# LCSL/nys-koop-lqr

Measured on AMD Instinct MI355X. Metric: Nyström-Koopman fits/sec (K_nm build + A,B,C solve), N=1e5 m=2000 d=384, higher is better.
Workload: dtype f64

## Files before the change

### nys_koop_lqr_amd/csrc/nk_api.hip

```cpp
#include "nk_common.h"

#include <cmath>
#include <cstdarg>
#include <cstdio>
#include <cstring>
#include <chrono>
#include <cstdlib>
#include <algorithm>
#include <condition_variable>
#include <mutex>
#include <set>
#include <thread>

namespace nk {

static thread_local std::string g_err;

void set_error(const char* fmt, ...) {
  char buf[1024];
  va_list ap;
  va_start(ap, fmt);
  vsnprintf(buf, sizeof(buf), fmt, ap);
  va_end(ap);
  g_err = buf;
// ... 792 lines not shown
        nk_model_destroy(m);
      }
    }
  } guard{ctx, mdl};
  mdl->ktype = kd->type; mdl->sigma0 = kd->sigma0; mdl->jitter = jitter;

  tr.mark("validate + model_alloc");
  hipEvent_t* ev = ctx->ev;
  NK_HIP(hipEventRecord(ev[0], ctx->stream));
  NK_TRY(make_winv(ctx, kd, d, mdl->winv));
  MatIn x, y, zi, zo;
  int host_passes = 1;
  if (mode != FIT_SOLVE) {
    const char* e = getenv("NYSKOOP_HOST_PASSES");
    const int want = e ? atoi(e) : 6;
    if (want > 1 && rng.size() == 2 && !ctx_recording(ctx) && (double)n_eff * (2.0 * d + p) * 8.0 >= 64e6 &&
        !is_device_ptr(X) && !is_device_ptr(Y))
      host_passes = want > 8 ? 8 : want;
  }
  if (mode != FIT_SOLVE && host_passes > 1) {
    x.ld = (d + p + 1) & ~(int64_t)1;
    y.ld = (d + 1) & ~(int64_t)1;
    double *xd = nullptr, *yd = nullptr;
    NK_TRY(arena_alloc_t(ctx, (size_t)n * x.ld, &xd));
    NK_TRY(arena_alloc_t(ctx, (size_t)n * y.ld, &yd));
    x.ptr = xd; y.ptr = yd; x.staged = y.staged = true;
  } else if (mode != FIT_SOLVE) {
    NK_TRY(stage_in(ctx, X, ldx, n, d + p, &x));
    NK_TRY(stage_in(ctx, Y, ldy, n, d, &y));
  }
  if (mode != FIT_SOLVE && rng.size() > 2 && (double)n_eff * (2.0 * d + p) * 8.0 <= 256e6) {
    const int64_t ldxg = (d + p + 1) & ~(int64_t)1, ldyg = (d + 1) & ~(int64_t)1;
    double *xg = nullptr, *yg = nullptr;
    NK_TRY(arena_alloc_t(ctx, (size_t)n_eff * ldxg, &xg));
    NK_TRY(arena_alloc_t(ctx, (size_t)n_eff * ldyg, &yg));
    int64_t o = 0;
    for (size_t i = 0; i < rng.size(); i += 2) {
      const int64_t b = rng[i], len = rng[i + 1] - rng[i];
      NK_TRY(launch_copy2d(ctx, x.ptr + b * x.ld, x.ld, xg + o * ldxg, ldxg, len, d + p));
      NK_TRY(launch_copy2d(ctx, y.ptr + b * y.ld, y.ld, yg + o * ldyg, ldyg, len, d));
      o += len;
    }
    x.ptr = xg; x.ld = ldxg; y.ptr = yg; y.ld = ldyg;
    rng.assign({(int64_t)0, n_eff});
  }
  NK_TRY(stage_in(ctx, Zout, ldzo, m, d, &zo));
  if (same_centers) zi = zo; else NK_TRY(stage_in(ctx, Zin, ldzi, m, d, &zi));
  NK_TRY(launch_copy2d(ctx, zo.ptr, zo.ld, mdl->Z, d, m, d));
  NK_HIP(hipEventRecord(ev[1], ctx->stream));
  tr.mark("staging issued");

  double *Kmm = nullptr, *Kj = nullptr, *Kj_in = nullptr, *Kxo = nullptr;
  bool landmarks_aside = false;
  if (mode != FIT_GRAM) {
  NK_TRY(arena_alloc_t(ctx, (size_t)m * m, &Kmm));
  NK_TRY(arena_alloc_t(ctx, (size_t)m * m, &Kj));
  if (same_centers) {
    Kj_in = Kj;
    Kxo = Kmm;
  } else {
    NK_TRY(arena_alloc_t(ctx, (size_t)m * m, &Kj_in));
    NK_TRY(arena_alloc_t(ctx, (size_t)m * m, &Kxo));
  }
  {
    const char* la = getenv("NYSKOOP_LANDMARKS_ASIDE");
    landmarks_aside = mode == FIT_FULL && n_eff >= 20000 && m >= 1024 && !ctx_recording(ctx) && !(la && la[0] == '0');
  }
  {
    hipStream_t s0 = ctx->stream;
    if (landmarks_aside) {
      NK_HIP(hipEventRecord(ev[12], ctx->stream));
      ctx->stream = ctx->stream_prep;
      NK_HIP(hipStreamWaitEvent(ctx->stream, ev[12], 0));
    }
    int rc_l = launch_kmat(ctx, kd->type, zo.ptr, zo.ld, m, zo.ptr, zo.ld, m, d, mdl->winv, kd->sigma0, Kmm, m);
    if (rc_l == NK_OK) rc_l = launch_copy2d(ctx, Kmm, m, Kj, m, m, m);
    if (rc_l == NK_OK) rc_l = launch_add_diag(ctx, Kj, m, m, jitter);
    if (rc_l == NK_OK && !same_centers) {
      rc_l = launch_kmat(ctx, kd->type, zi.ptr, zi.ld, m, zi.ptr, zi.ld, m, d, mdl->winv, kd->sigma0, Kj_in, m);
      if (rc_l == NK_OK) rc_l = launch_add_diag(ctx, Kj_in, m, m, jitter);
      if (rc_l == NK_OK) rc_l = launch_kmat(ctx, kd->type, zi.ptr, zi.ld, m, zo.ptr, zo.ld, m, d, mdl->winv, kd->sigma0, Kxo, m);
    }
    const hipError_t he = rc_l == NK_OK ? hipEventRecord(ev[8], ctx->stream) : hipSuccess;
    ctx->stream = s0;
    NK_TRY(rc_l);
    NK_HIP(he);
  }
  }
  double *G1 = nullptr, *G2 = nullptr, *G3 = nullptr, *G4 = nullptr;
  const int64_t ldd = d + (d & 1);
  NK_TRY(arena_alloc_t(ctx, gram_doubles(m, d, p), &G1));
  G2 = G1 + (size_t)mp * mp;
  G3 = G1 + gram_block1(m, p);
  G4 = G3 + (size_t)m * m;
  float ms_gram_kernel = 0.f;
  int gram_launches = 0;
  bool gram_deferred = false;
  const bool timed = stats != nullptr;
  SqrtPlan splan;
  int it = 0;
  double resid = 0.0;
  double *Sinvt = nullptr, *T1t = nullptr, *X1 = nullptr;
  auto alloc_sqrt_bufs = [&]() -> int {
    if (Sinvt == nullptr) NK_TRY(arena_alloc_t(ctx, (size_t)m * m, &Sinvt));
    if (T1t == nullptr) NK_TRY(arena_alloc_t(ctx, (size_t)m * m, &T1t));
    if (X1 == nullptr) NK_TRY(arena_alloc_t(ctx, (size_t)m * m, &X1));
    return NK_OK;
  };
  auto sqrt_products = [&]() -> int {
    NK_TRY(launch_transpose(ctx, mdl->Sinv, m, Sinvt, m, m, m));
    if (same_centers) {
      NK_TRY(launch_copy2d(ctx, mdl->S, m, T1t, m, m, m));
      NK_TRY(launch_axpby2d(ctx, -jitter, mdl->Sinv, m, 1.0, T1t, m, m, m));
    } else {
      NK_TRY(launch_transpose(ctx, Kxo, m, X1, m, m, m));
      NK_TRY(launch_gemm(ctx, true, false, m, m, m, 1.0, X1, m, mdl->Sinv, m, 0.0, T1t, m));
    }
    return NK_OK;
  };
  auto queue_prep = [&]() -> int {
    SideScope prep(ctx, ctx->stream_prep);
    NK_HIP(hipStreamWaitEvent(ctx->stream, ev[8], 0));
    splan.lambda_min_hint = jitter > 0.0 ? jitter : 0.0;
    if (mode == FIT_FULL && n_eff >= 20000 && m >= 1024) {
      static const double frac = getenv("NYSKOOP_PREP_PAUSE") ? atof(getenv("NYSKOOP_PREP_PAUSE")) : 0.0;
      const int nb = (m + CHOL_NB - 1) / CHOL_NB;
      if (frac < 1.0) {
        splan.pause_event = ctx->ev_fork;
        splan.pause_step = std::max(0, std::min(nb - 1, (int)(frac * nb)));
      }
    }
    NK_TRY(sqrtm_prepare(ctx, Kj, m, m, &splan));
    NK_HIP(hipEventRecord(ev[9], ctx->stream));
    return NK_OK;
  };
  auto queue_side = [&]() -> int {
    NK_TRY(alloc_sqrt_bufs());
    SideScope side(ctx);
    NK_HIP(hipStreamWaitEvent(ctx->stream, ctx->ev_fork, 0));
    NK_HIP(hipStreamWaitEvent(ctx->stream, ev[9], 0));
    NK_HIP(hipEventRecord(ev[6], ctx->stream));
    NK_TRY(sqrtm_finish(ctx, &splan, mdl->S, mdl->Sinv));
    NK_HIP(hipEventRecord(ev[7], ctx->stream));
    NK_TRY(sqrt_products());
    NK_HIP(hipEventRecord(ctx->ev_join, ctx->stream));
    return NK_OK;
  };
  if (mode == FIT_SOLVE) {
    NK_HIP(hipMemcpyAsync(G1, gram_io, gram_doubles(m, d, p) * sizeof(double),
                          is_device_ptr(gram_io) ? hipMemcpyDeviceToDevice : hipMemcpyHostToDevice, ctx->stream));
    NK_HIP(hipEventRecord(ev[2], ctx->stream));
  } else {
  const bool f32 = ctx->compute_f32 != 0 && ctx->kmat_mode == 0 && d >= 32 && !ctx_recording(ctx) && m >= 4 && d >= 4;
  const int64_t off_out = f32 ? ((mp + 3) & ~3) : ((mp + 1) & ~1);
  const int64_t ldf = f32 ? ((off_out + m + 3) & ~(int64_t)3) : ((off_out + m + 1) & ~(int64_t)1);
  const double felem = f32 ? 4.0 : 8.0;
  int64_t pass_rows;
  {
    const char* b = getenv("NYSKOOP_F_BUDGET_GB");
    const double budget = (b ? atof(b) : 48.0) * 1073741824.0;
    pass_rows = (int64_t)(budget / ((double)ldf * felem));
    if (pass_rows < 1024) pass_rows = 1024;
    pass_rows &= ~(int64_t)1023;
    if (host_passes > 1) {
      const int64_t per = ((n_eff + host_passes - 1) / host_passes + 1023) & ~(int64_t)1023;
      if (per < pass_rows) pass_rows = per;
    }
  }
  struct Piece { int64_t b, len; };
  std::vector<std::vector<Piece>> passes(1);
  {
    int64_t used = 0;
    for (size_t i = 0; i < rng.size(); i += 2) {
      int64_t b = rng[i];
      const int64_t e = rng[i + 1];
      while (b < e) {
        if (used == pass_rows) { passes.emplace_back(); used = 0; }
        const int64_t len = std::min(e - b, pass_rows - used);
        passes.back().push_back(Piece{b, len});
        used += len;
        b += len;
      }
    }
  }
  const int64_t f_rows = passes.size() > 1 ? pass_rows : n_eff;
  double* F = nullptr;
  NK_TRY(arena_alloc_t(ctx, f32 ? ((size_t)f_rows * ldf + 1) / 2 + 64 : (size_t)f_rows * ldf + 64, &F));
  const bool gram_form = ctx->kmat_mode == 0 && d >= 32;
  int64_t maxlen = 0;
  for (auto& ps : passes) for (auto& pc : ps) maxlen = std::max(maxlen, pc.len);
  const int64_t ldt = (maxlen + 1) & ~(int64_t)1, ldzt = (m + 1) & ~1;
  double *center = nullptr, *Rt = nullptr, *sqr = nullptr, *Zto = nullptr, *sqzo = nullptr, *Zti = nullptr, *sqzi = nullptr;
  double *Rt2 = nullptr, *sqr2 = nullptr;
  const bool overlap_prep = gram_form && passes.size() == 1 && passes[0].size() == 1;
  if (gram_form) {
    NK_TRY(arena_alloc_t(ctx, (size_t)d, &center));
    if (!f32) {
      NK_TRY(arena_alloc_t(ctx, (size_t)d * ldt, &Rt));
      NK_TRY(arena_alloc_t(ctx, (size_t)maxlen, &sqr));
    }
    if (overlap_prep && !f32) {
      NK_TRY(arena_alloc_t(ctx, (size_t)d * ldt, &Rt2));
      NK_TRY(arena_alloc_t(ctx, (size_t)maxlen, &sqr2));
    }
    NK_TRY(arena_alloc_t(ctx, (size_t)d * ldzt, &Zto));
    NK_TRY(arena_alloc_t(ctx, (size_t)m, &sqzo));
    if (kd->type == NK_KERNEL_LINEAR) NK_TRY(launch_fill(ctx, center, d, 1, d, 0.0));
    else NK_TRY(launch_colmean(ctx, zo.ptr, zo.ld, m, d, center));
    NK_TRY(prep_rows(ctx, zo.ptr, zo.ld, m, d, mdl->winv, center, Zto, ldzt, sqzo));
    if (same_centers) {
      Zti = Zto; sqzi = sqzo;
    } else {
      NK_TRY(arena_alloc_t(ctx, (size_t)d * ldzt, &Zti));
      NK_TRY(arena_alloc_t(ctx, (size_t)m, &sqzi));
      NK_TRY(prep_rows(ctx, zi.ptr, zi.ld, m, d, mdl->winv, center, Zti, ldzt, sqzi));
    }
  }
  float *F32 = reinterpret_cast<float*>(F), *Rt32 = nullptr, *sq32 = nullptr, *Zt32 = nullptr, *sqz32 = nullptr, *Y32 = nullptr;
  const int64_t ldt32 = (maxlen + 3) & ~(int64_t)3, ldzt32 = (m + 3) & ~3, ldy32 = (d + 3) & ~3;
  if (f32) {
    NK_REQUIRE(same_centers, "fp32 engine: separate input landmarks are not supported");
    double* tmp = nullptr;
    NK_TRY(arena_alloc_t(ctx, ((size_t)d * ldt32 + 1) / 2 + 2, &tmp)); Rt32 = reinterpret_cast<float*>(tmp);
    NK_TRY(arena_alloc_t(ctx, ((size_t)maxlen + 1) / 2 + 2, &tmp)); sq32 = reinterpret_cast<float*>(tmp);
    NK_TRY(arena_alloc_t(ctx, ((size_t)d * ldzt32 + 1) / 2 + 2, &tmp)); Zt32 = reinterpret_cast<float*>(tmp);
    NK_TRY(arena_alloc_t(ctx, ((size_t)m + 1) / 2 + 2, &tmp)); sqz32 = reinterpret_cast<float*>(tmp);
    NK_TRY(arena_alloc_t(ctx, ((size_t)f_rows * ldy32 + 1) / 2 + 2, &tmp)); Y32 = reinterpret_cast<float*>(tmp);
    NK_TRY(prep_rows_f32(ctx, zo.ptr, zo.ld, m, d, mdl->winv, center, Zt32, ldzt32, sqz32));
  }
  const bool multi_pass = passes.size() > 1;
  const bool pipelined = host_passes > 1;
  auto upload_pass = [&](size_t ip) -> int {
    for (const Piece& pc : passes[ip]) {
      NK_HIP(hipMemcpy2DAsync(const_cast<double*>(x.ptr) + pc.b * x.ld, (size_t)x.ld * 8, X + pc.b * ldx, (size_t)ldx * 8,
                              (size_t)(d + p) * 8, (size_t)pc.len, hipMemcpyHostToDevice, ctx->stream_side));
      NK_HIP(hipMemcpy2DAsync(const_cast<double*>(y.ptr) + pc.b * y.ld, (size_t)y.ld * 8, Y + pc.b * ldy, (size_t)ldy * 8,
                              (size_t)d * 8, (size_t)pc.len, hipMemcpyHostToDevice, ctx->stream_side));
    }
    NK_HIP(hipEventRecord(ctx->ev_up[ip & 7], ctx->stream_side));
    return NK_OK;
  };
  if (pipelined) {
    NK_HIP(hipEventRecord(ev[12], ctx->stream));
    NK_HIP(hipStreamWaitEvent(ctx->stream_side, ev[12], 0));
    NK_TRY(upload_pass(0));
  }
  for (size_t ip = 0; ip < passes.size(); ++ip) {
    const std::vector<Piece>& ps = passes[ip];
    const double beta = ip == 0 ? 0.0 : 1.0;
    if (pipelined) NK_HIP(hipStreamWaitEvent(ctx->stream, ctx->ev_up[ip & 7], 0));
    if (f32) {
      int64_t o32 = 0;
      for (const Piece& pc : ps) {
        const double* xs = x.ptr + pc.b * x.ld;
        const double* ys = y.ptr + pc.b * y.ld;
        NK_TRY(prep_rows_f32(ctx, xs, x.ld, pc.len, d, mdl->winv, center, Rt32, ldt32, sq32));
        NK_TRY(launch_kmat_gram_f32(ctx, kd->type, Rt32, ldt32, sq32, pc.len, Zt32, ldzt32, sqz32, m, d, kd->sigma0,
                                    F32 + o32 * ldf, ldf));
        NK_TRY(prep_rows_f32(ctx, ys, y.ld, pc.len, d, mdl->winv, center, Rt32, ldt32, sq32));
        NK_TRY(launch_kmat_gram_f32(ctx, kd->type, Rt32, ldt32, sq32, pc.len, Zt32, ldzt32, sqz32, m, d, kd->sigma0,
                                    F32 + o32 * ldf + off_out, ldf));
        if (p > 0) NK_TRY(launch_cvt_f64_f32(ctx, xs + d, x.ld, F32 + o32 * ldf + m, ldf, pc.len, p));
        NK_TRY(launch_cvt_f64_f32(ctx, ys, y.ld, Y32 + o32 * ldy32, ldy32, pc.len, d));
        o32 += pc.len;
      }
      if (ip == 0) {
        NK_HIP(hipEventRecord(ev[2], ctx->stream));
        tr.mark("kmat issued");
      }
      TnProblemF pf[4];
      pf[0].A = F32; pf[0].B = F32; pf[0].lda = pf[0].ldb = ldf; pf[0].M = pf[0].N = mp; pf[0].C = G1; pf[0].ldc = mp;
      pf[0].tri = TRI_UPPER_MIRROR;
      pf[1].A = F32 + off_out; pf[1].B = F32; pf[1].lda = pf[1].ldb = ldf; pf[1].M = m; pf[1].N = mp; pf[1].C = G2; pf[1].ldc = mp;
      pf[2].A = F32 + off_out; pf[2].B = F32 + off_out; pf[2].lda = pf[2].ldb = ldf; pf[2].M = pf[2].N = m; pf[2].C = G3;
      pf[2].ldc = m; pf[2].tri = TRI_UPPER_MIRROR;
      pf[3].A = Y32; pf[3].lda = ldy32; pf[3].M = d; pf[3].N = m; pf[3].C = G4; pf[3].ldc = m; pf[3].B = F32 + off_out;
      pf[3].ldb = ldf;
      for (int q = 0; q < 4; ++q) pf[q].beta = beta;
      float ms1 = 0.f;
      NK_TRY(launch_gemm_tn_f32_multi(ctx, pf, 4, o32, 0, timed ? &ms1 : nullptr, multi_pass));
      if (multi_pass) ms_gram_kernel += ms1; else gram_deferred = timed;
      gram_launches += 1;
      if (pipelined && ip + 1 < passes.size()) NK_TRY(upload_pass(ip + 1));
      continue;
    }
    int64_t o = 0;
    for (const Piece& pc : ps) {
      const double* xs = x.ptr + pc.b * x.ld;
      const double* ys = y.ptr + pc.b * y.ld;
      if (gram_form && overlap_prep) {
        NK_HIP(hipEventRecord(ev[12], ctx->stream));
        {
          SideScope side(ctx);
          NK_HIP(hipStreamWaitEvent(ctx->stream, ev[12], 0));
          NK_TRY(prep_rows(ctx, ys, y.ld, pc.len, d, mdl->winv, center, Rt2, ldt, sqr2));
          NK_HIP(hipEventRecord(ev[13], ctx->stream));
        }
        NK_TRY(prep_rows(ctx, xs, x.ld, pc.len, d, mdl->winv, center, Rt, ldt, sqr));
        NK_TRY(launch_kmat_gram(ctx, kd->type, Rt, ldt, sqr, pc.len, Zti, ldzt, sqzi, m, d, kd->sigma0, F + o * ldf, ldf));
        NK_HIP(hipStreamWaitEvent(ctx->stream, ev[13], 0));
        NK_TRY(launch_kmat_gram(ctx, kd->type, Rt2, ldt, sqr2, pc.len, Zto, ldzt, sqzo, m, d, kd->sigma0,
                                F + o * ldf + off_out, ldf));
      } else if (gram_form) {
        NK_TRY(prep_rows(ctx, xs, x.ld, pc.len, d, mdl->winv, center, Rt, ldt, sqr));
        NK_TRY(launch_kmat_gram(ctx, kd->type, Rt, ldt, sqr, pc.len, Zti, ldzt, sqzi, m, d, kd->sigma0, F + o * ldf, ldf));
        NK_TRY(prep_rows(ctx, ys, y.ld, pc.len, d, mdl->winv, center, Rt, ldt, sqr));
        NK_TRY(launch_kmat_gram(ctx, kd->type, Rt, ldt, sqr, pc.len, Zto, ldzt, sqzo, m, d, kd->sigma0,
                                F + o * ldf + off_out, ldf));
      } else {
        NK_TRY(launch_kmat(ctx, kd->type, xs, x.ld, pc.len, zi.ptr, zi.ld, m, d, mdl->winv, kd->sigma0, F + o * ldf, ldf));
        NK_TRY(launch_kmat(ctx, kd->type, ys, y.ld, pc.len, zo.ptr, zo.ld, m, d, mdl->winv, kd->sigma0,
                           F + o * ldf + off_out, ldf));
      }
      if (p > 0) NK_TRY(launch_copy2d(ctx, xs + d, x.ld, F + o * ldf + m, ldf, pc.len, p));
      o += pc.len;
    }
    const int64_t rows = o;
    if (ip == 0) {
      NK_HIP(hipEventRecord(ev[2], ctx->stream));
      tr.mark("kmat issued");
    }
    TnProblem pr[4];
    pr[0].A = F; pr[0].B = F; pr[0].lda = pr[0].ldb = ldf; pr[0].M = pr[0].N = mp; pr[0].C = G1; pr[0].ldc = mp;
    pr[0].tri = TRI_UPPER_MIRROR;
    pr[1].A = F + off_out; pr[1].B = F; pr[1].lda = pr[1].ldb = ldf; pr[1].M = m; pr[1].N = mp; pr[1].C = G2;
    pr[1].ldc = mp;
    pr[2].A = F + off_out; pr[2].B = F + off_out; pr[2].lda = pr[2].ldb = ldf; pr[2].M = pr[2].N = m; pr[2].C = G3;
    pr[2].ldc = m; pr[2].tri = TRI_UPPER_MIRROR;
    pr[3].A = y.ptr + ps[0].b * y.ld; pr[3].lda = y.ld; pr[3].M = d; pr[3].N = m; pr[3].C = G4; pr[3].ldc = m;
    pr[3].B = F + off_out; pr[3].ldb = ldf;
    for (int q = 0; q < 4; ++q) pr[q].beta = beta;
    const bool single = ps.size() == 1;
    const bool fast = tn_fast_ok(pr[0]) && tn_fast_ok(pr[1]) && tn_fast_ok(pr[2]);
    const bool fast_y = fast && tn_fast_ok(pr[3]);
    bool y_done = false;
    if (fast) {
      const int np = (single && fast_y) ? 4 : 3;
      float ms1 = 0.f;
      NK_TRY(launch_gemm_tn_multi(ctx, pr, np, rows, 0, (timed && !pipelined) ? &ms1 : nullptr, multi_pass));
      if (multi_pass) ms_gram_kernel += ms1; else gram_deferred = timed;
      gram_launches += 1;
      y_done = np == 4;
    } else {
      GemmOpts sym;
      sym.tri = TRI_UPPER_MIRROR;
      float t3[3] = {0.f, 0.f, 0.f};
      NK_TRY(launch_gemm(ctx, true, false, mp, mp, rows, 1.0, F, ldf, F, ldf, beta, G1, mp, sym, timed ? &t3[0] : nullptr));
      NK_TRY(launch_gemm(ctx, true, false, m, mp, rows, 1.0, F + off_out, ldf, F, ldf, beta, G2, mp, GemmOpts(),
                         timed ? &t3[1] : nullptr));
      NK_TRY(launch_gemm(ctx, true, false, m, m, rows, 1.0, F + off_out, ldf, F + off_out, ldf, beta, G3, m, sym,
                         timed ? &t3[2] : nullptr));
      ms_gram_kernel += t3[0] + t3[1] + t3[2];
      gram_launches += 3;
    }
    if (!y_done) {
      int64_t oo = 0;
      bool first = true;
      for (const Piece& pc : ps) {
        NK_TRY(launch_gemm(ctx, true, false, d, m, pc.len, 1.0, y.ptr + pc.b * y.ld, y.ld, F + oo * ldf + off_out, ldf,
                           (first && ip == 0) ? 0.0 : 1.0, G4, m));
        oo += pc.len;
        first = false;
      }
    }
    if (pipelined && ip + 1 < passes.size()) NK_TRY(upload_pass(ip + 1));
  }
  }
  NK_HIP(hipEventRecord(ev[3], ctx->stream));
  if (mode == FIT_GRAM) {
    NK_HIP(hipMemcpyAsync(gram_io, G1, gram_doubles(m, d, p) * sizeof(double),
                          is_device_ptr(gram_io) ? hipMemcpyDeviceToDevice : hipMemcpyDeviceToHost, ctx->stream));
    NK_HIP(hipStreamSynchronize(ctx->stream));
    if (stats) {
      memset(stats, 0, sizeof(*stats));
      stats->ms_total = ev_ms(ctx, 0, 3);
      stats->ms_upload = (x.staged || y.staged) ? ev_ms(ctx, 0, 1) : 0.0;
      stats->ms_kmat = ev_ms(ctx, 1, 2);
      stats->ms_gram = ev_ms(ctx, 2, 3);
      if (gram_deferred) ms_gram_kernel = ev_ms(ctx, 14, 15);
      stats->ms_gram_kernel_avg = gram_launches ? ms_gram_kernel / gram_launches : 0.0;
      stats->gram_kernel_launches = gram_launches;
    }
    if (ctx->arena.chunks.size() > 1 || ctx->arena_side.chunks.size() > 1) NK_TRY(arena_reset(ctx));
    return NK_OK;
  }
  NK_HIP(hipEventRecord(ctx->ev_fork, ctx->stream));
  tr.mark("gram issued");

  NK_TRY(queue_prep());

  if (landmarks_aside) NK_HIP(hipStreamWaitEvent(ctx->stream, ev[8], 0));
  NK_TRY(launch_axpby2d(ctx, gamma_n, Kj_in, m, 1.0, G1, mp, m, m));
  if (p > 0) NK_TRY(launch_add_diag(ctx, G1 + (int64_t)m * mp + m, mp, p, gamma_n));
  NK_TRY(launch_axpby2d(ctx, gamma_n, Kj, m, 1.0, G3, m, m, m));
  double* Gsave = nullptr;
  NK_TRY(arena_alloc_t(ctx, gram_doubles(m, d, p), &Gsave));
  NK_HIP(hipMemcpyAsync(Gsave, G1, gram_doubles(m, d, p) * sizeof(double), hipMemcpyDeviceToDevice, ctx->stream));
  double *Linv = nullptr, *Linv2 = nullptr, *V1 = nullptr, *Wc = nullptr, *Ct = nullptr;
  const int nblk = (mp + CHOL_NB - 1) / CHOL_NB;
  NK_TRY(arena_alloc_t(ctx, (size_t)nblk * CHOL_WS, &Linv));
  NK_TRY(arena_alloc_t(ctx, (size_t)nblk * CHOL_WS, &Linv2));
  NK_TRY(arena_alloc_t(ctx, (size_t)m * m, &V1));
  NK_TRY(alloc_sqrt_bufs());
  NK_TRY(arena_alloc_t(ctx, (size_t)m * ldd, &Wc));
  NK_TRY(arena_alloc_t(ctx, (size_t)m * ldd, &Ct));
  CholSys sys[2];
  double* pivlog = nullptr;
  NK_TRY(arena_alloc_t(ctx, (size_t)mp + m + 4, &pivlog));
  sys[0].P = G1; sys[0].ldp = mp; sys[0].m = mp; sys[0].Linv = Linv; sys[0].extra = m;
  sys[1].P = G3; sys[1].ldp = m; sys[1].m = m; sys[1].Linv = Linv2; sys[1].extra = d;
  sys[0].pivlog = pivlog; sys[1].pivlog = pivlog + mp + (mp & 1);
  NK_TRY(cholesky_aug_pair_async(ctx, sys, 2));
  tr.mark("cholesky + solves issued");

  NK_TRY(queue_side());
  NK_HIP(hipStreamWaitEvent(ctx->stream, ctx->ev_join, 0));
  NK_HIP(hipEventRecord(ev[4], ctx->stream));
  tr.mark("side stream joined (queued)");

  auto operator_products = [&]() -> int {
    NK_TRY(launch_transpose(ctx, G2, mp, V1, m, m, m));
    NK_TRY(launch_gemm(ctx, true, false, m, m, m, 1.0, V1, m, T1t, m, 0.0, X1, m));
    NK_TRY(launch_gemm(ctx, true, false, m, m, m, 1.0, Sinvt, m, X1, m, 0.0, mdl->A, mp));
    if (p > 0) NK_TRY(launch_gemm(ctx, true, false, m, p, m, 1.0, Sinvt, m, G2 + m, mp, 0.0, mdl->B, mp));
    NK_TRY(launch_transpose(ctx, G4, m, Wc, ldd, d, m));
    NK_TRY(launch_gemm(ctx, true, false, m, d, m, 1.0, mdl->S, m, Wc, ldd, 0.0, Ct, ldd));
    NK_TRY(launch_transpose(ctx, Ct, ldd, mdl->C, m, m, d));
    NK_TRY(launch_gemm(ctx, true, false, d, mp, m, 1.0, Ct, ldd, mdl->A, mp, 0.0, mdl->W, mp));
    return NK_OK;
  };
  NK_TRY(operator_products());
  NK_HIP(hipEventRecord(ev[5], ctx->stream));
  tr.mark("solve issued");
  int chol_failed[2] = {0, 0};
  double piv_ratio[2] = {1.0, 1.0};
  NK_TRY(cholesky_fail_flags(ctx, sys, 2, chol_failed, piv_ratio));
  tr.mark("final sync");
  bool chol_rerun = false;
  if (chol_failed[0] == CHOL_FLOW_GIVEUP || chol_failed[1] == CHOL_FLOW_GIVEUP) {
    ChainOnly chain(ctx);
    NK_HIP(hipMemcpyAsync(G1, Gsave, gram_doubles(m, d, p) * sizeof(double), hipMemcpyDeviceToDevice, ctx->stream));
    NK_TRY(cholesky_aug_pair_async(ctx, sys, 2));
// ... 894 lines not shown
```

### nys_koop_lqr_amd/csrc/nk_chol_flow.hip

```cpp
#include "nk_common.h"
#include "nk_panel_body.h"
#include "nk_potrf_body.h"

namespace nk {

namespace {

constexpr int FLOW_THREADS = 256;
constexpr int FLOW_HDR = 16;
constexpr int FLOW_POLL_LIMIT = 1 << 22;

struct FlowSys {
  double* P;
  int64_t ldp;
  int m, extra;
  double* Linv;
  double* pivlog;
  int* info;
  unsigned long long* piv;
  int* flags;
  int nblk;
  int nex;
};
struct FlowArgs {
// ... 209 lines not shown
          if (J < 0) { ok = false; break; }
          for (; j < J; ++j) {
            update_quarter(s, r0, r1, p0, c0, j, wm, wn, l15, l4, Cp);
            update_quarter(s, r0, r1, c0, c1, j, wm, wn, l15, l4, Cd);
          }
        }
        if (!ok) continue;
        store_quarter(s, r0, r1, p0, c0, wm, wn, l15, l4, Cp);
        store_quarter(s, r0, r1, c0, c1, wm, wn, l15, l4, Cd);
        local_sync();
        if (wait_tiles(a, s, k - 1, -1, k - 1, k, sh) < 0) continue;
        panel_tile(a, s, r0, r1, k - 1, wave, lane);
        publish(s, k, k - 1);
        __syncthreads();
        load_quarter(s, r0, r1, c0, c1, wm, wn, l15, l4, Cd);
        update_quarter(s, r0, r1, c0, c1, k - 1, wm, wn, l15, l4, Cd);
        store_quarter(s, r0, r1, c0, c1, wm, wn, l15, l4, Cd);
        local_sync();
      }
      if (wave == 0)
        flow_potrf(s.P + (int64_t)c0 * s.ldp + c0, s.ldp, c1 - c0, s.Linv + (size_t)k * CHOL_WS, s.info, s.piv,
                   s.pivlog ? s.pivlog + c0 : nullptr, k, lane);
      publish(s, k, k);
      __syncthreads();
    } else {
      if (k > 0) {
        Quarter C;
        load_quarter(s, r0, r1, c0, c1, wm, wn, l15, l4, C);
        bool ok = true;
        for (int j = 0; j < k && ok;) {
          const int J = wait_tiles(a, s, i, k, j, k, sh);
          if (J < 0) { ok = false; break; }
          for (; j < J; ++j) update_quarter(s, r0, r1, c0, c1, j, wm, wn, l15, l4, C);
        }
        if (!ok) continue;
        store_quarter(s, r0, r1, c0, c1, wm, wn, l15, l4, C);
        local_sync();
      }
      if (wait_tiles(a, s, k, -1, k, k + 1, sh) < 0) continue;
      panel_tile(a, s, r0, r1, k, wave, lane);
      publish(s, i, k);
      __syncthreads();
    }
  }
}

}

bool chol_flow_enabled() {
  const char* e = getenv("NYSKOOP_CHOL_FLOW");
  return !(e && e[0] == '0');
}

int cholesky_flow_pair(nk_ctx* ctx, const CholSys* sys, int nsys) {
  constexpr int NB = CHOL_NB;
  NK_REQUIRE(nsys >= 1 && nsys <= 2, "cholesky_flow_pair: 1..2 systems");
  FlowArgs a;
  memset(&a, 0, sizeof(a));
  a.nsys = nsys;
  a.fix = chol_fix_enabled();
  size_t words = FLOW_HDR;
  for (int q = 0; q < nsys; ++q) {
    const CholSys& y = sys[q];
    FlowSys& s = a.s[q];
    s.P = y.P; s.ldp = y.ldp; s.m = y.m; s.extra = y.extra; s.Linv = y.Linv; s.pivlog = y.pivlog;
    s.info = ctx->d_info + info_base(ctx) + q;
    s.piv = ctx->d_piv + 2 * (info_base(ctx) + q);
    s.nblk = (y.m + NB - 1) / NB;
    s.nex = (y.extra + NB - 1) / NB;
    words += (size_t)(s.nblk + s.nex) * s.nblk;
    for (int c = 0; c < s.nblk; ++c) a.total += 1 + std::max(0, s.nblk - c - 2) + s.nex;
  }
  const int slot = info_base(ctx) / 2;
  if (ctx->flow_words[slot] < words) {
    if (ctx->d_flow[slot]) NK_HIP(hipFree(ctx->d_flow[slot]));
    ctx->d_flow[slot] = nullptr;
    ctx->flow_words[slot] = 0;
    NK_HIP(hipMalloc(reinterpret_cast<void**>(&ctx->d_flow[slot]), words * sizeof(int)));
    ctx->flow_words[slot] = words;
  }
  a.hdr = ctx->d_flow[slot];
  int* f = a.hdr + FLOW_HDR;
  for (int q = 0; q < nsys; ++q) {
    a.s[q].flags = f;
    f += (size_t)(a.s[q].nblk + a.s[q].nex) * a.s[q].nblk;
  }
  NK_HIP(hipMemsetAsync(a.hdr, 0, words * sizeof(int), ctx->stream));
  const int grid = std::max(1, std::min(a.total, ctx->num_cu / 2));
  hipLaunchKernelGGL(chol_flow_kernel, dim3((unsigned)grid), dim3(FLOW_THREADS), 0, ctx->stream, a);
  NK_HIP(hipGetLastError());
  count_event(CNT_CHOL_FLOW);
  return NK_OK;
}

}
```

### nys_koop_lqr_amd/csrc/nk_common.h

```cpp
#pragma once
#include <hip/hip_runtime.h>
#include <stdint.h>
#include <stddef.h>
#include <string>
#include <vector>

#include "nyskoop.h"
#include "nk_lockstep.h"

namespace nk {

void set_error(const char* fmt, ...);

#define NK_HIP(call)                                                                         \
  do {                                                                                       \
    hipError_t e_ = (call);                                                                  \
    if (e_ != hipSuccess) {                                                                  \
      nk::set_error("%s failed: %s (%s:%d)", #call, hipGetErrorString(e_), __FILE__, __LINE__); \
      return e_ == hipErrorOutOfMemory ? NK_ERR_OOM : NK_ERR_HIP;                            \
    }                                                                                        \
  } while (0)

#define NK_TRY(call)            \
  do {                          \
// ... 159 lines not shown
enum { TRI_FULL = 0, TRI_UPPER_MIRROR = 1, TRI_LOWER = 2 };
struct GemmOpts {
  int tri = TRI_FULL;
  int splitk = 0;
};
int launch_gemm(nk_ctx* ctx, bool transA, bool transB, int64_t M, int64_t N, int64_t K, double alpha, const double* A,
                int64_t lda, const double* B, int64_t ldb, double beta, double* C, int64_t ldc,
                const GemmOpts& opts = GemmOpts(), float* ms_kernel = nullptr);

struct GemmCall {
  int64_t M = 0, N = 0, K = 0;
  double alpha = 1.0, beta = 0.0;
  const double* A = nullptr;
  const double* B = nullptr;
  double* C = nullptr;
  int64_t lda = 0, ldb = 0, ldc = 0;
  GemmOpts opts;
};
int launch_gemm_pair(nk_ctx* ctx, bool transA, bool transB, const GemmCall* calls, int ncalls);

struct TnSkip;
int launch_add_diag(nk_ctx* ctx, double* A, int64_t lda, int n, double v);
int launch_copy2d(nk_ctx* ctx, const double* src, int64_t lds, double* dst, int64_t ldd, int64_t rows, int64_t cols);
int launch_axpby2d(nk_ctx* ctx, double a, const double* X, int64_t ldx, double b, double* Y, int64_t ldy,
                   int64_t rows, int64_t cols);
int launch_scale_add_identity(nk_ctx* ctx, double a, const double* X, int64_t ldx, double c, double* Y, int64_t ldy,
                              int n, const TnSkip* skip = nullptr);
int launch_fill(nk_ctx* ctx, double* A, int64_t lda, int64_t rows, int64_t cols, double v);
int launch_frob_minus_identity(nk_ctx* ctx, const double* M, int64_t ldm, int n, double* d_out,
                               const TnSkip* skip = nullptr);
int launch_max_abs_rowsum(nk_ctx* ctx, const double* M, int64_t ldm, int n, double* d_out);
int launch_colsum_sqdiff(nk_ctx* ctx, const double* P, int64_t ldp, const double* Y, int64_t ldy, int64_t rows,
                         int cols, double* d_colsum);

int sqrtm_spd(nk_ctx* ctx, const double* P, int64_t ldp, int m, double* S, double* Sinv, int* iters, double* resid);
struct SqrtPlan {
  const double* P = nullptr;
  int64_t ldp = 0;
  int m = 0;
  double* W = nullptr;
  double* Linv = nullptr;
  double* X0 = nullptr;
  double* X0t = nullptr;
  double* d_sc = nullptr;
  ArenaMark mark{0, 0};
  bool deferred = false;
  int rc = 0, iters = 0, kmax = 0;
  double resid = 0.0;
  double lambda_min_hint = 0.0;
  bool early = false;
  bool flow_gave_up = false;
  hipEvent_t pause_event = nullptr;
  int pause_step = -1;
};
constexpr int NK_SQRT_RETRY = 1;
int sqrtm_spd_coupled(nk_ctx* ctx, const double* P, int64_t ldp, int m, double* S, double* Sinv, int* iters, double* resid);
int sqrtm_prepare(nk_ctx* ctx, const double* P, int64_t ldp, int m, SqrtPlan* plan);
int sqrtm_finish(nk_ctx* ctx, SqrtPlan* plan, double* S, double* Sinv);
int sqrtm_verdict(nk_ctx* ctx, SqrtPlan* plan, int* iters, double* resid);
int cholesky_lower(nk_ctx* ctx, double* P, int64_t ldp, int m, double* Linv );
int cholesky_solve(nk_ctx* ctx, const double* L, int64_t ldl, int m, const double* Linv, double* R, int64_t ldr,
                   int nrhs);
struct CholSys {
  double* P = nullptr;
  int64_t ldp = 0;
  int m = 0;
  int extra = 0;
  bool backward = true;
  double* Linv = nullptr;
  double* pivlog = nullptr;
  double* R = nullptr;
  int64_t ldr = 0;
  int nrhs = 0;
};
int cholesky_lower_pair(nk_ctx* ctx, const CholSys* sys, int nsys);
int cholesky_lower_pair_async(nk_ctx* ctx, const CholSys* sys, int nsys);
int cholesky_check_pair(nk_ctx* ctx, const CholSys* sys, int nsys);
int cholesky_solve_pair(nk_ctx* ctx, const CholSys* sys, int nsys);
int cholesky_aug_pair_async(nk_ctx* ctx, const CholSys* sys, int nsys, hipEvent_t pause = nullptr, int pause_step = -1);
constexpr int CHOL_NB = 64;
constexpr int CHOL_WS = 2 * CHOL_NB * CHOL_NB + 8;
constexpr double CHOL_FIX_KAPPA = 8.0 * CHOL_NB;
inline int chol_fix_enabled() {
  const char* e = getenv("NYSKOOP_CHOL_FIX");
  return (e && e[0] == '0') ? 0 : ((e && e[0] == '2') ? 2 : 1);
}
bool launch_chol_trail_pair(nk_ctx* ctx, const GemmCall* calls, int ncalls, int* rc);
bool launch_chol_trail_potrf_pair(nk_ctx* ctx, const GemmCall* calls, int ncalls, const int* nb, double* const* Linv, int blk,
                                  double* const* plog, int* rc);
inline bool chol_fuse_enabled() {
  const char* e = getenv("NYSKOOP_CHOL_FUSE");
  return !(e && e[0] == '0');
}
bool chol_flow_enabled();
int cholesky_flow_pair(nk_ctx* ctx, const CholSys* sys, int nsys);
constexpr int CHOL_FLOW_GIVEUP = -0x40000000;
bool launch_chol_panel_pair(nk_ctx* ctx, const GemmCall* calls, int ncalls, int* rc);
int launch_trsm_right_lower_pair(nk_ctx* ctx, const CholSys* sys, int nsys);

struct PinvInfo {
  int rank = 0, sweeps = 0;
  bool converged = false;
  double sigma_max = 0.0, sigma_min_kept = 0.0, sigma_min = 0.0;
};
int pinv_right_divide(nk_ctx* ctx, const double* P, int64_t ldp, int m, const double* E, int64_t lde, int rows,
                      double* E_out, int64_t ldeo, double rcond, PinvInfo* info);
int cholesky_fail_flags(nk_ctx* ctx, const CholSys* sys, int nsys, int* failed , double* piv_ratio = nullptr);

int launch_lifted_step(nk_ctx* ctx, const double* G, int64_t ldg, int m, int mz, int pu, const double* z, int64_t zstride,
                       const double* u, int64_t ustride, const double* bias, double* out, int64_t ostride, int batch);

struct ChainArgs {
  const double* G = nullptr; int64_t ldg = 0; int m = 0, pu = 0;
  const double* z0 = nullptr; int64_t z0_stride = 0;
  bool lift = false;
  const double* x0 = nullptr; int64_t x0_stride = 0;
  const double* Zl = nullptr; int d = 0; const double* winv = nullptr; const double* Sinv = nullptr; int ktype = 0;
  double sigma0 = 0.0;
  const double* U = nullptr; int64_t u_stride = 0;
  const double* bias = nullptr; int64_t bias_stride = 0;
  double* Zall = nullptr; int64_t z_stride = 0;
  int T = 0, batch = 0;
};
int launch_ref_minus_traj(nk_ctx* ctx, const double* ref, int64_t ref_stride, const double* Phi, int64_t phi_stride,
                          double* D, int64_t d_stride, int steps, int m, int batch);
bool lifted_chain_ok(int m, int pu, int d_lift);
int launch_lifted_chain(nk_ctx* ctx, const ChainArgs& a);
bool lifted_chain_mw_ok(const nk_ctx* ctx, int m, int pu);
int chain_mw_workgroups(int m);
int chain_mw_group(int m, int batch);
int launch_lifted_chain_mw(nk_ctx* ctx, const ChainArgs& a);
int lifted_chain_mw_reset(nk_ctx* ctx);
int lifted_chain_mw_fetch_status(nk_ctx* ctx);
bool lifted_chain_mw_timed_out(nk_ctx* ctx, int* row, int* step, int* traj);

}

namespace nk {
enum { KTRIM_NONE = 0, KTRIM_B_UPPER = 1 , KTRIM_A_LOWER = 2  };
struct TnProblem {
  const double* A = nullptr;
  const double* B = nullptr;
  double* C = nullptr;
  int64_t lda = 0, ldb = 0, ldc = 0;
  int M = 0, N = 0;
  int tri = TRI_FULL;
  int ktrim = 0;
  double alpha = 1.0, beta = 0.0;
// ... 85 lines not shown
```

### nys_koop_lqr_amd/csrc/nk_linalg.hip

```cpp
#include "nk_common.h"

#include <algorithm>
#include <cmath>
#include <cstring>
#include <vector>

namespace nk {

__device__ __forceinline__ void add_diag_kernel_body(double* A, int64_t lda, int n, double v) {
  int i = blockIdx.x * blockDim.x + threadIdx.x;
  if (i < n) A[(int64_t)i * lda + i] += v;
}
__global__ void __launch_bounds__(256) add_diag_kernel(double* A, int64_t lda, int n, double v) { add_diag_kernel_body(A, lda, n, v); }
NK_BATCHED_TWIN(add_diag_kernel, (256), double*, int64_t, int, double)
__device__ __forceinline__ void copy2d_kernel_body(const double* __restrict__ src, int64_t lds, double* __restrict__ dst, int64_t ldd, int64_t rows, int64_t cols) {
  const int64_t total = rows * cols;
  for (int64_t e = blockIdx.x * (int64_t)blockDim.x + threadIdx.x; e < total; e += (int64_t)gridDim.x * blockDim.x) {
    const int64_t r = e / cols, c = e - r * cols;
    dst[r * ldd + c] = src[r * lds + c];
  }
}
__global__ void __launch_bounds__(256) copy2d_kernel(const double* __restrict__ src, int64_t lds, double* __restrict__ dst, int64_t ldd, int64_t rows, int64_t cols) { copy2d_kernel_body(src, lds, dst, ldd, rows, cols); }
NK_BATCHED_TWIN(copy2d_kernel, (256), const double*, int64_t, double*, int64_t, int64_t, int64_t)
__device__ __forceinline__ void axpby2d_kernel_body(double a, const double* __restrict__ X, int64_t ldx, double b, double* __restrict__ Y, int64_t ldy, int64_t rows, int64_t cols) {
// ... 592 lines not shown
      if (failed[q] > 0)
        set_error("Cholesky: non-positive pivot at index %d of %d (system %d is numerically rank deficient; the "
                  "reference's lstsq would truncate here)", failed[q] - 1, sys[q].m, q);
      else
        set_error("Cholesky: system %d (order %d) has an isolated cluster of rounding-level pivots: an exact null space (the "
                  "reference's lstsq truncates it)", q, sys[q].m);
      return NK_ERR_NOT_SPD;
    }
  return NK_OK;
}

int cholesky_fail_flags(nk_ctx* ctx, const CholSys* sys, int nsys, int* failed, double* piv_ratio) {
  const int ib = info_base(ctx);
  std::vector<double> plog[2];
  NK_HIP(hipMemcpyAsync(ctx->h_info + ib, ctx->d_info + ib, 2 * sizeof(int), hipMemcpyDeviceToHost, ctx->stream));
  NK_HIP(hipMemcpyAsync(ctx->h_piv + 2 * ib, ctx->d_piv + 2 * ib, 4 * sizeof(unsigned long long), hipMemcpyDeviceToHost,
                        ctx->stream));
  for (int q = 0; q < nsys; ++q)
    if (sys[q].pivlog) {
      plog[q].resize((size_t)sys[q].m);
      NK_HIP(hipMemcpyAsync(plog[q].data(), sys[q].pivlog, sizeof(double) * sys[q].m, hipMemcpyDeviceToHost, ctx->stream));
    }
  NK_HIP(hipStreamSynchronize(ctx->stream));
  const double eps = 2.220446049250313e-16;
  for (int q = 0; q < nsys; ++q) {
    failed[q] = ctx->h_info[ib + q];
    if (piv_ratio) piv_ratio[q] = 0.0;
    if (failed[q] == CHOL_FLOW_GIVEUP) {
      if (q == 0) count_event(CNT_CHOL_FLOW_GIVEUP);
      continue;
    }
    if (failed[q] != 0) continue;
    double dmin, dmax;
    memcpy(&dmin, &ctx->h_piv[2 * (ib + q)], 8);
    memcpy(&dmax, &ctx->h_piv[2 * (ib + q) + 1], 8);
    if (!(dmax > 0.0)) continue;
    if (piv_ratio) piv_ratio[q] = dmin / dmax;
    if (dmin <= eps * dmax) { failed[q] = -1; continue; }
    if (plog[q].empty()) continue;
    std::sort(plog[q].begin(), plog[q].end());
    const double window = 8.0 * (double)sys[q].m * eps * dmax;
    size_t k = 0;
    while (k < plog[q].size() && plog[q][k] <= window) ++k;
    if (k > 0 && k < plog[q].size() && plog[q][k] >= 1000.0 * plog[q][k - 1]) failed[q] = -1;
  }
  return NK_OK;
}

int cholesky_lower_pair(nk_ctx* ctx, const CholSys* sys, int nsys) {
  NK_TRY(cholesky_lower_pair_async(ctx, sys, nsys));
  return cholesky_check_pair(ctx, sys, nsys);
}

int cholesky_aug_pair_async(nk_ctx* ctx, const CholSys* sys, int nsys, hipEvent_t pause, int pause_step) {
  constexpr int NB = CHOL_NB;
  NK_REQUIRE(nsys >= 1 && nsys <= 2, "cholesky_aug_pair: 1..2 systems");
  NK_TRY(reset_pivots(ctx));
  int nblk = 0, mmin = sys[0].m;
  for (int q = 0; q < nsys; ++q) {
    nblk = std::max(nblk, (sys[q].m + NB - 1) / NB);
    mmin = std::min(mmin, sys[q].m);
  }
  if (!ctx->chol_flow_off && mmin >= 256 && !ctx_recording(ctx) && chol_flow_enabled()) {
    if (pause != nullptr && pause_step >= 0 && pause_step < nblk) NK_HIP(hipStreamWaitEvent(ctx->stream, pause, 0));
    NK_TRY(cholesky_flow_pair(ctx, sys, nsys));
    NK_TRY(launch_trsm_right_lower_pair(ctx, sys, nsys));
    return NK_OK;
  }
  static const bool la_env = getenv("NYSKOOP_CHOL_LOOKAHEAD") && getenv("NYSKOOP_CHOL_LOOKAHEAD")[0] == '1';
  const int la = ctx->stream == ctx->stream_main ? 1 : -1;
  const bool lookahead = la_env && la >= 0 && nblk >= 4 && !ctx_recording(ctx);
  hipStream_t s_chain = ctx->stream;
  hipStream_t s_rest = lookahead ? ctx->stream_la[la] : ctx->stream;
  hipEvent_t* ev = lookahead ? ctx->ev_la[la] : nullptr;
  bool rest_pending = false;
  hipEvent_t last_rest = nullptr;
  if (lookahead) {
    NK_HIP(hipEventRecord(ev[1], s_chain));
    NK_HIP(hipStreamWaitEvent(s_rest, ev[1], 0));
  }
  const bool fuse = chol_fuse_enabled();
  bool diag_done = false;
  for (int jb = 0; jb < nblk; ++jb) {
    if (pause != nullptr && jb == pause_step) NK_HIP(hipStreamWaitEvent(ctx->stream, pause, 0));
    const int j0 = jb * NB;
    double* Ajj[2] = {nullptr, nullptr};
    double* Li[2] = {nullptr, nullptr};
    double* Pl[2] = {nullptr, nullptr};
    int64_t lda[2] = {0, 0};
    int nbj[2] = {0, 0};
    GemmCall panel[2], trail[2], next[2], rest[2];
    bool any_rest = false;
    for (int q = 0; q < nsys; ++q) {
      const CholSys& y = sys[q];
      if (j0 >= y.m) continue;
      nbj[q] = y.m - j0 < NB ? y.m - j0 : NB;
      Ajj[q] = y.P + (int64_t)j0 * y.ldp + j0;
      lda[q] = y.ldp;
      Li[q] = y.Linv + (size_t)jb * CHOL_WS;
      Pl[q] = y.pivlog ? y.pivlog + j0 : nullptr;
      const int rem = y.m - j0 - nbj[q];
      const int rows = rem + y.extra;
      if (rows > 0) {
        double* pnl = y.P + (int64_t)(j0 + nbj[q]) * y.ldp + j0;
        panel[q].M = rows; panel[q].N = nbj[q]; panel[q].K = nbj[q];
        panel[q].A = pnl; panel[q].lda = y.ldp; panel[q].B = Li[q]; panel[q].ldb = NB;
        panel[q].C = pnl; panel[q].ldc = y.ldp;
        if (rem > 0) {
          trail[q].M = rows; trail[q].N = rem; trail[q].K = nbj[q]; trail[q].alpha = -1.0; trail[q].beta = 1.0;
          trail[q].A = pnl; trail[q].lda = y.ldp; trail[q].B = pnl; trail[q].ldb = y.ldp;
          trail[q].C = y.P + (int64_t)(j0 + nbj[q]) * y.ldp + (j0 + nbj[q]); trail[q].ldc = y.ldp;
          trail[q].opts.tri = TRI_LOWER;
          const int nbn = rem < NB ? rem : NB;
          next[q] = trail[q];
          next[q].N = nbn;
          if (rem > nbn) {
            rest[q] = trail[q];
            rest[q].M = rows - nbn; rest[q].N = rem - nbn;
// ... 136 lines not shown
}

__device__ __forceinline__ void tri_scale_both_kernel_body(const double* __restrict__ L, int64_t ldl, int m, const double* __restrict__ d_c, double* __restrict__ Xt, double* __restrict__ X) {
  __shared__ double tile[32][33];
  const double s = 1.0 / sqrt(d_c[0]);
  const int bx = blockIdx.x * 32, by = blockIdx.y * 32;
  const int tx = threadIdx.x & 31, ty = threadIdx.x >> 5;
  for (int r = ty; r < 32; r += 8) {
    const int i = by + r, j = bx + tx;
    double v = 0.0;
    if (i < m && j <= i) v = L[(int64_t)i * ldl + j] * s;
    if (i < m && j < m) Xt[(int64_t)i * m + j] = v;
    tile[r][tx] = v;
  }
  __syncthreads();
  for (int r = ty; r < 32; r += 8) {
    const int i = bx + r, j = by + tx;
    if (i < m && j < m) X[(int64_t)i * m + j] = tile[tx][r];
  }
}
__global__ void __launch_bounds__(256) tri_scale_both_kernel(const double* __restrict__ L, int64_t ldl, int m, const double* __restrict__ d_c, double* __restrict__ Xt, double* __restrict__ X) { tri_scale_both_kernel_body(L, ldl, m, d_c, Xt, X); }
NK_BATCHED_TWIN(tri_scale_both_kernel, (256), const double*, int64_t, int, const double*, double*, double*)

int sqrtm_prepare(nk_ctx* ctx, const double* P, int64_t ldp, int m, SqrtPlan* plan) {
  plan->P = P; plan->ldp = ldp; plan->m = m;
  plan->mark = arena_mark(ctx);
  const size_t mm = (size_t)m * m;
  const int nblk = (m + CHOL_NB - 1) / CHOL_NB;
  NK_TRY(arena_alloc_t(ctx, 2 * mm, &plan->W));
  NK_TRY(arena_alloc_t(ctx, (size_t)nblk * CHOL_WS, &plan->Linv));
  NK_TRY(arena_alloc_t(ctx, mm, &plan->X0));
  NK_TRY(arena_alloc_t(ctx, mm, &plan->X0t));
  NK_TRY(arena_alloc_t(ctx, (size_t)8, &plan->d_sc));
  NK_TRY(launch_max_abs_rowsum(ctx, P, ldp, m, plan->d_sc));
  {
    const ArenaMark mk = arena_mark(ctx);
    const int blocks = grid_for((int64_t)m * m, ctx->num_cu);
    double* partial = nullptr;
    NK_TRY(arena_alloc_t(ctx, (size_t)2 * blocks, &partial));
    hipLaunchKernelGGL(sumsq_trace_partial_kernel, dim3(blocks), dim3(256), 0, ctx->stream, P, ldp, m, partial, blocks);
    hipLaunchKernelGGL(sum_partials_kernel, dim3(1), dim3(256), 0, ctx->stream, partial, blocks, plan->d_sc + 1);
    hipLaunchKernelGGL(sum_partials_kernel, dim3(1), dim3(256), 0, ctx->stream, partial + blocks, blocks, plan->d_sc + 2);
    NK_HIP(hipGetLastError());
    arena_release(ctx, mk);
  }
  NK_HIP(hipMemcpyAsync(ctx->h_scalars + 12, plan->d_sc, 3 * sizeof(double), hipMemcpyDeviceToHost, ctx->stream));
  NK_HIP(hipEventRecord(ctx->ev[11], ctx->stream));
  double* E = plan->W + mm;
  NK_TRY(launch_copy2d(ctx, P, ldp, plan->W, m, m, m));
  NK_TRY(launch_fill(ctx, E, m, m, m, 0.0));
  NK_TRY(launch_add_diag(ctx, E, m, m, 1.0));
  CholSys y;
  y.P = plan->W; y.ldp = m; y.m = m; y.extra = m; y.backward = false; y.Linv = plan->Linv;
  NK_TRY(cholesky_aug_pair_async(ctx, &y, 1, plan->pause_event, plan->pause_step));
  {
    const ArenaMark mk = arena_mark(ctx);
    const int blocks = grid_for((int64_t)m * m, ctx->num_cu);
    double* partial = nullptr;
    NK_TRY(arena_alloc_t(ctx, (size_t)2 * blocks, &partial));
    hipLaunchKernelGGL(sumsq_trace_partial_kernel, dim3(blocks), dim3(256), 0, ctx->stream, E, (int64_t)m, m, partial, blocks);
    hipLaunchKernelGGL(sum_partials_kernel, dim3(1), dim3(256), 0, ctx->stream, partial, blocks, plan->d_sc + 3);
    NK_HIP(hipGetLastError());
    arena_release(ctx, mk);
  }
  const int tb = (m + 31) / 32;
  hipLaunchKernelGGL(tri_scale_both_kernel, dim3(tb, tb), dim3(256), 0, ctx->stream, plan->W, (int64_t)m, m, plan->d_sc,
                     plan->X0t, plan->X0);
  NK_HIP(hipGetLastError());
  return NK_OK;
}

__device__ __forceinline__ void ns_flag_kernel_body(const double* __restrict__ partial, int count, int m, int step, double* __restrict__ state) {
  __shared__ double sh[4];
  double s = 0.0;
  for (int i = threadIdx.x; i < count; i += blockDim.x) s += partial[i];
  s = wave_sum(s);
  if ((threadIdx.x & 63) == 0) sh[threadIdx.x >> 6] = s;
  __syncthreads();
  if (threadIdx.x == 0) {
    const double r = sqrt((sh[0] + sh[1] + sh[2] + sh[3]) / m);
    state[2] = r;
    if (state[0] == 0.0 && r < 1e-7) {
      state[0] = (double)(step + 1);
      state[1] = r;
    }
  }
}
__global__ void __launch_bounds__(256) ns_flag_kernel(const double* __restrict__ partial, int count, int m, int step, double* __restrict__ state) { ns_flag_kernel_body(partial, count, m, step, state); }
NK_BATCHED_TWIN(ns_flag_kernel, (256), const double*, int, int, int, double*)

static int sqrtm_polar_products(nk_ctx* ctx, SqrtPlan* plan, const double* Q, double* scratch, double c, double* S,
                                double* Sinv, const double* Q_even = nullptr, const double* select = nullptr) {
  const int m = plan->m;
  const size_t mm = (size_t)m * m;
  double* Linv_full = scratch;
  NK_TRY(launch_transpose(ctx, plan->W + mm, m, Linv_full, m, m, m));
  TnProblem pr[2];
  pr[0].A = Q; pr[0].B = plan->X0; pr[0].C = S; pr[0].lda = pr[0].ldb = pr[0].ldc = m; pr[0].M = pr[0].N = m;
  pr[0].alpha = std::sqrt(c);
  pr[0].ktrim = KTRIM_B_UPPER;
  pr[1].ktrim = KTRIM_A_LOWER;
  pr[1].A = Linv_full; pr[1].B = Q; pr[1].C = Sinv; pr[1].lda = pr[1].ldb = pr[1].ldc = m; pr[1].M = pr[1].N = m;
  pr[0].A_even = Q_even;
  pr[1].B_even = Q_even;
  TnSkip sel;
  sel.select = select;
  if (tn_fast_ok(pr[0]) && tn_fast_ok(pr[1]) && m >= 128) {
// ... 248 lines not shown
```

Measured before the change: 24.49.

## Issue K_mm sqrt prep before the gram build and overlap with a narrower flow grid

```diff
diff --git a/nys_koop_lqr_amd/csrc/nk_api.hip b/nys_koop_lqr_amd/csrc/nk_api.hip
--- a/nys_koop_lqr_amd/csrc/nk_api.hip
+++ b/nys_koop_lqr_amd/csrc/nk_api.hip
@@ -868,6 +868,8 @@
 
   double *Kmm = nullptr, *Kj = nullptr, *Kj_in = nullptr, *Kxo = nullptr;
   bool landmarks_aside = false;
+  bool kmm_early = false;
+  int kmm_grid = 0;
   if (mode != FIT_GRAM) {
   NK_TRY(arena_alloc_t(ctx, (size_t)m * m, &Kmm));
   NK_TRY(arena_alloc_t(ctx, (size_t)m * m, &Kj));
@@ -938,7 +940,8 @@
     SideScope prep(ctx, ctx->stream_prep);
     NK_HIP(hipStreamWaitEvent(ctx->stream, ev[8], 0));
     splan.lambda_min_hint = jitter > 0.0 ? jitter : 0.0;
-    if (mode == FIT_FULL && n_eff >= 20000 && m >= 1024) {
+    splan.flow_grid = kmm_early ? kmm_grid : 0;
+    if (!kmm_early && mode == FIT_FULL && n_eff >= 20000 && m >= 1024) {
       static const double frac = getenv("NYSKOOP_PREP_PAUSE") ? atof(getenv("NYSKOOP_PREP_PAUSE")) : 0.0;
       const int nb = (m + CHOL_NB - 1) / CHOL_NB;
       if (frac < 1.0) {
@@ -1000,6 +1003,17 @@
     }
   }
   const int64_t f_rows = passes.size() > 1 ? pass_rows : n_eff;
+  {
+    const char* ke = getenv("NYSKOOP_KMM_EARLY");
+    kmm_early = mode == FIT_FULL && n_eff >= 20000 && m >= 1024 && passes.size() == 1 && !ctx_recording(ctx) &&
+                !ctx->chol_flow_off && chol_flow_enabled() && !(ke && ke[0] == '0');
+    kmm_grid = std::max(1, (ke && ke[0] == '2') ? ctx->num_cu / 2 : ctx->num_cu / 4);
+  }
+  if (kmm_early) NK_TRY(queue_prep());
+  auto gate_gram = [&]() -> int {
+    if (kmm_early) NK_HIP(hipStreamWaitEvent(ctx->stream, ev[9], 0));
+    return NK_OK;
+  };
   double* F = nullptr;
   NK_TRY(arena_alloc_t(ctx, f32 ? ((size_t)f_rows * ldf + 1) / 2 + 64 : (size_t)f_rows * ldf + 64, &F));
   const bool gram_form = ctx->kmat_mode == 0 && d >= 32;
@@ -1081,6 +1095,7 @@
         o32 += pc.len;
       }
       if (ip == 0) {
+        NK_TRY(gate_gram());
         NK_HIP(hipEventRecord(ev[2], ctx->stream));
         tr.mark("kmat issued");
       }
@@ -1133,6 +1148,7 @@
     }
     const int64_t rows = o;
     if (ip == 0) {
+      NK_TRY(gate_gram());
       NK_HIP(hipEventRecord(ev[2], ctx->stream));
       tr.mark("kmat issued");
     }
@@ -1203,7 +1219,7 @@
   NK_HIP(hipEventRecord(ctx->ev_fork, ctx->stream));
   tr.mark("gram issued");
 
-  NK_TRY(queue_prep());
+  if (!kmm_early) NK_TRY(queue_prep());
 
   if (landmarks_aside) NK_HIP(hipStreamWaitEvent(ctx->stream, ev[8], 0));
   NK_TRY(launch_axpby2d(ctx, gamma_n, Kj_in, m, 1.0, G1, mp, m, m));
diff --git a/nys_koop_lqr_amd/csrc/nk_chol_flow.hip b/nys_koop_lqr_amd/csrc/nk_chol_flow.hip
--- a/nys_koop_lqr_amd/csrc/nk_chol_flow.hip
+++ b/nys_koop_lqr_amd/csrc/nk_chol_flow.hip
@@ -285,7 +285,7 @@
   return !(e && e[0] == '0');
 }
 
-int cholesky_flow_pair(nk_ctx* ctx, const CholSys* sys, int nsys) {
+int cholesky_flow_pair(nk_ctx* ctx, const CholSys* sys, int nsys, int grid_req) {
   constexpr int NB = CHOL_NB;
   NK_REQUIRE(nsys >= 1 && nsys <= 2, "cholesky_flow_pair: 1..2 systems");
   FlowArgs a;
@@ -319,7 +319,7 @@
     f += (size_t)(a.s[q].nblk + a.s[q].nex) * a.s[q].nblk;
   }
   NK_HIP(hipMemsetAsync(a.hdr, 0, words * sizeof(int), ctx->stream));
-  const int grid = std::max(1, std::min(a.total, ctx->num_cu / 2));
+  const int grid = std::max(1, std::min(a.total, grid_req > 0 ? grid_req : ctx->num_cu / 2));
   hipLaunchKernelGGL(chol_flow_kernel, dim3((unsigned)grid), dim3(FLOW_THREADS), 0, ctx->stream, a);
   NK_HIP(hipGetLastError());
   count_event(CNT_CHOL_FLOW);
diff --git a/nys_koop_lqr_amd/csrc/nk_common.h b/nys_koop_lqr_amd/csrc/nk_common.h
--- a/nys_koop_lqr_amd/csrc/nk_common.h
+++ b/nys_koop_lqr_amd/csrc/nk_common.h
@@ -235,6 +235,7 @@
   bool flow_gave_up = false;
   hipEvent_t pause_event = nullptr;
   int pause_step = -1;
+  int flow_grid = 0;
 };
 constexpr int NK_SQRT_RETRY = 1;
 int sqrtm_spd_coupled(nk_ctx* ctx, const double* P, int64_t ldp, int m, double* S, double* Sinv, int* iters, double* resid);
@@ -260,7 +261,8 @@
 int cholesky_lower_pair_async(nk_ctx* ctx, const CholSys* sys, int nsys);
 int cholesky_check_pair(nk_ctx* ctx, const CholSys* sys, int nsys);
 int cholesky_solve_pair(nk_ctx* ctx, const CholSys* sys, int nsys);
-int cholesky_aug_pair_async(nk_ctx* ctx, const CholSys* sys, int nsys, hipEvent_t pause = nullptr, int pause_step = -1);
+int cholesky_aug_pair_async(nk_ctx* ctx, const CholSys* sys, int nsys, hipEvent_t pause = nullptr, int pause_step = -1,
+                            int flow_grid = 0);
 constexpr int CHOL_NB = 64;
 constexpr int CHOL_WS = 2 * CHOL_NB * CHOL_NB + 8;
 constexpr double CHOL_FIX_KAPPA = 8.0 * CHOL_NB;
@@ -276,7 +278,7 @@
   return !(e && e[0] == '0');
 }
 bool chol_flow_enabled();
-int cholesky_flow_pair(nk_ctx* ctx, const CholSys* sys, int nsys);
+int cholesky_flow_pair(nk_ctx* ctx, const CholSys* sys, int nsys, int grid = 0);
 constexpr int CHOL_FLOW_GIVEUP = -0x40000000;
 bool launch_chol_panel_pair(nk_ctx* ctx, const GemmCall* calls, int ncalls, int* rc);
 int launch_trsm_right_lower_pair(nk_ctx* ctx, const CholSys* sys, int nsys);
diff --git a/nys_koop_lqr_amd/csrc/nk_linalg.hip b/nys_koop_lqr_amd/csrc/nk_linalg.hip
--- a/nys_koop_lqr_amd/csrc/nk_linalg.hip
+++ b/nys_koop_lqr_amd/csrc/nk_linalg.hip
@@ -668,7 +668,7 @@
   return cholesky_check_pair(ctx, sys, nsys);
 }
 
-int cholesky_aug_pair_async(nk_ctx* ctx, const CholSys* sys, int nsys, hipEvent_t pause, int pause_step) {
+int cholesky_aug_pair_async(nk_ctx* ctx, const CholSys* sys, int nsys, hipEvent_t pause, int pause_step, int flow_grid) {
   constexpr int NB = CHOL_NB;
   NK_REQUIRE(nsys >= 1 && nsys <= 2, "cholesky_aug_pair: 1..2 systems");
   NK_TRY(reset_pivots(ctx));
@@ -679,7 +679,7 @@
   }
   if (!ctx->chol_flow_off && mmin >= 256 && !ctx_recording(ctx) && chol_flow_enabled()) {
     if (pause != nullptr && pause_step >= 0 && pause_step < nblk) NK_HIP(hipStreamWaitEvent(ctx->stream, pause, 0));
-    NK_TRY(cholesky_flow_pair(ctx, sys, nsys));
+    NK_TRY(cholesky_flow_pair(ctx, sys, nsys, flow_grid));
     NK_TRY(launch_trsm_right_lower_pair(ctx, sys, nsys));
     return NK_OK;
   }
@@ -922,7 +922,7 @@
   NK_TRY(launch_add_diag(ctx, E, m, m, 1.0));
   CholSys y;
   y.P = plan->W; y.ldp = m; y.m = m; y.extra = m; y.backward = false; y.Linv = plan->Linv;
-  NK_TRY(cholesky_aug_pair_async(ctx, &y, 1, plan->pause_event, plan->pause_step));
+  NK_TRY(cholesky_aug_pair_async(ctx, &y, 1, plan->pause_event, plan->pause_step, plan->flow_grid));
   {
     const ArenaMark mk = arena_mark(ctx);
     const int blocks = grid_for((int64_t)m * m, ctx->num_cu);
```

Result: faster. 24.78, median of 6 (+1.2%).
